# vdBerg93/cl-rrt

Hardware: AMD Instinct MI355X
Metric: nodes expanded/sec (200-obstacle scene) (higher is better)
Workload: dtype f64

## Files before the change

cl-rrt_amd/clrrt/__init__.py:

```python
import ctypes as C
import os

import numpy as np

from . import abi
from .abi import (CLRRT_COLLISION_OBB, CLRRT_COLLISION_STUB, CLRRT_MODE_BATCH,
                  CLRRT_MODE_EXACT, ROLL_NAMES)

PKG_DIR = os.path.dirname(os.path.dirname(os.path.abspath(__file__)))
LIB_PATH = os.environ.get("CLRRT_LIB") or os.path.join(PKG_DIR, "libclrrt.so")
HEADER_PATH = os.path.join(os.path.dirname(PKG_DIR), "include", "clrrt.h")

_lib = None
P = C.POINTER
EXCHANGE_FN = C.CFUNCTYPE(C.c_int32, C.c_void_p, P(abi.ExchangeIO))

_SIGS = {
    "clrrt_abi_version": (C.c_int, []),
    "clrrt_params_default": (C.c_int, [P(abi.Params), C.c_double, P(C.c_double), C.c_double]),
    "clrrt_rng_seed": (None, [P(abi.Rng), C.c_uint32]),
    "clrrt_rng_next": (C.c_int32, [P(abi.Rng)]),
    "clrrt_draw_samples": (C.c_int, [P(abi.Params), P(abi.Rng), C.c_int32, P(abi.Sample)]),
    "clrrt_create": (C.c_int, [P(abi.Params), P(abi.Capacity), C.c_int, P(C.c_void_p)]),
    "clrrt_destroy": (None, [C.c_void_p]),
# ... 486 lines not shown
        self._chk(self.L.clrrt_exact_stats(self.h, out), "exact_stats")
        return dict(zip(("rounds", "resolved", "fixup_rollouts", "conflict_rounds", "end_fixup_succeeded", "end_tie",
                         "end_key_eq_thr", "end_over_slots", "end_pushed_out"), list(out)[:9]))

    def iteration_log(self, on=True):
        self._chk(self.L.clrrt_iteration_log(self.h, 1 if on else 0), "iteration_log")

    def iterations(self):
        n = C.c_int64()
        self._chk(self.L.clrrt_iteration_records(self.h, 0, 0, None, C.byref(n)), "iteration_records")
        arr = (abi.Iteration * max(1, n.value))()
        self._chk(self.L.clrrt_iteration_records(self.h, 0, n.value, arr, C.byref(n)), "iteration_records")
        return {f: np.array([getattr(arr[i], f) for i in range(n.value)], dtype=np.int64)
                for f, _ in abi.Iteration._fields_}

    def round_sizes(self):
        n = C.c_int64()
        self._chk(self.L.clrrt_round_sizes(self.h, None, 0, C.byref(n)), "round_sizes")
        out = np.zeros(max(1, n.value), dtype=np.int64)
        self._chk(self.L.clrrt_round_sizes(self.h, out.ctypes.data_as(P(C.c_int64)), n.value, C.byref(n)), "round_sizes")
        return out[:n.value]

    def walk_audit(self, samples):
        n = len(samples)
        arr = (abi.Sample * n)(*samples)
        out = np.zeros((n, 20), dtype=np.int32)
        self._chk(self.L.clrrt_walk_audit(self.h, arr, n, out.ctypes.data_as(P(C.c_int32))), "walk_audit")
        return out

    def search_work_ex(self):
        out = (C.c_int64 * 8)()
        self._chk(self.L.clrrt_search_work_ex(self.h, out), "search_work_ex")
        return {"bf_keys": out[0], "samples": out[1], "tiles": out[2], "exact_keys": out[3],
                "super_bounds": out[4], "super_visits": out[5], "queued": out[6]}

    def reset_counters(self):
        self._chk(self.L.clrrt_reset_counters(self.h), "reset_counters")

    def enable_timing(self, on=True):
        self._chk(self.L.clrrt_enable_timing(self.h, 1 if on else 0), "enable_timing")

    def set_option(self, key, value):
        self._chk(self.L.clrrt_set_option(self.h, key.encode(), int(value)), f"set_option({key})")

    def nn_stats(self):
        out = (C.c_int64 * 19)()
        self._chk(self.L.clrrt_nn_stats(self.h, out), "nn_stats")
        return {"waves": out[0], "nodes_read": out[1], "rings": out[2], "truncated_waves": out[3],
                "last_fallback_samples": out[4], "tiles_seen": out[5], "tiles_searched": out[6],
                "pairs_queued": out[7], "exact_keys": out[8], "walk_supers": out[10], "walk_tiles": out[11],
                "walk_queued": out[12], "walk_exact": out[13], "walk_clk_bounds": out[14], "walk_clk_super": out[15],
                "walk_clk_visit": out[16], "walk_clk_drain": out[17], "walk_clk_total": out[18]}

    def debug_counters(self):
        out = (C.c_int64 * 64)()
        self._chk(self.L.clrrt_debug_counters(self.h, out), "debug_counters")
        return list(out)

    def kernel_time(self, which):
        ms, n = C.c_double(), C.c_int64()
        self._chk(self.L.clrrt_kernel_time(self.h, which, C.byref(ms), C.byref(n)), "kernel_time")
        return ms.value, n.value
```

cl-rrt_amd/csrc/clrrt_capi.hip:

```cpp
#include <hip/hip_runtime.h>
#include <math.h>

#include <algorithm>
#include <climits>
#include <array>
#include <chrono>
#include <cmath>
#include <cstdio>
#include <cstdlib>
#include <cstring>
#include <deque>
#include <functional>
#include <optional>
#include <string>
#include <vector>

#include "../../include/clrrt.h"
#include "clrrt_dev.hpp"
#include "clrrt_internal.hpp"

static const int kWalkMaxOver = 2048, kWalkMaxChunks = 64;

using namespace clrrt;

// ... 35 lines not shown
  KeyId* sort_scratch = nullptr;
  int64_t sort_cap = 0;
  RollRes* res_spec = nullptr;
  clrrt_node* regnodes = nullptr;
  RollRes* res_gb = nullptr;
  double* slots = nullptr;
  int slot_rows = 0;
  int rows_deferred = 1;
  void* rep_buf = nullptr;
  int rep_n = 0;
  bool eval_deferred = false;
  clrrt_node* gbnodes = nullptr;
  SampleOut* so = nullptr;
  int* first_conflict = nullptr;
  clrrt_node* out_nodes = nullptr;
  Job* jobs = nullptr;
  int64_t* totals = nullptr;
  bool totals_zeroed = false;
  unsigned long long* work_ctr = nullptr;
  float* nn_seed = nullptr;
  double bbox[4] = {HUGE_VAL, HUGE_VAL, -HUGE_VAL, -HUGE_VAL};
  double* d_bbox = nullptr;
  double* h_bbox = nullptr;
  int64_t nnw_min_nodes = 8192;
  bool nnw_stateless = false;
  int nnw_bud_tiles = 3072, nnw_bud_ex = 4096, nnw_chunks = 16, nnw_max_over = 1024;
  bool nnw_max_over_set = false;
  bool nnw_bud_tiles_set = false;
  int nnw_half_max = 4096;
  int nnw_hscale = 50;
  int nnw_lpt = 0;
  int nnw_root_seed = 1;
  int nnw_root_k = 64;
  int nnw_root_scan = 16384;
  int nnw_index = 5;
  int nnw_lds_floor = 0;
  int nnw_waves = -1;
  int nnw_double = 1;
  WalkBufs nnw{};
  WalkBufs nnw_alt{};
  struct { int64_t n = -1; double ox, oy, x0, y0, x1, y1; float delta; } nnw_built;
  CompactBufs cmp{};
  int roll_persistent = 1;
  int nn_debug = 0;
  int roll_blocks = 0;
  int n_cu = 256;
  int* roll_q = nullptr;
  int* roll_best = nullptr;
  int roll_priority = 1;
  int roll_order_verify = 0;
  int roll_coop = 1;
  int roll_spread = 1;
  int roll_lanes = 0;
  int nn_exact_fused = 1;
  int exact_min_width = 8;
  int exact_fixup = 1;
  int exact_fix_cap = 0;
  int* fix_n = nullptr;
  int* fix_ids = nullptr;
  int* fix_adj = nullptr;
  NnRec* fix_xrec = nullptr;
  int* fix_xi = nullptr;
  int* fix_xcand = nullptr;
  float* fix_xkey = nullptr;
  int* fix_xn = nullptr;
  std::vector<int> h_fix_cand;
// ... 1115 lines not shown
  HIPC(c, hipSetDevice(c->device));
  unsigned long long h[4];
  HIPC(c, hipMemcpyAsync(h, c->work_ctr, sizeof(h), hipMemcpyDeviceToHost, c->stream));
  HIPC(c, hipStreamSynchronize(c->stream));
  for (int i = 0; i < 3; i++) out[i] = (int64_t)h[i];
  return CLRRT_OK;
}

int clrrt_search_work(clrrt_ctx* c, int64_t out[4]) {
  if (!c || !out) return CLRRT_EINVAL;
  HIPC(c, hipSetDevice(c->device));
  HIPC(c, hipStreamSynchronize(c->stream));
  if (c->side) HIPC(c, hipStreamSynchronize(c->side));
  unsigned long long h[19];
  HIPC(c, hipMemcpy(h, c->work_ctr + 8, sizeof(h), hipMemcpyDeviceToHost));
  out[0] = c->nn_bf_keys;
  out[1] = c->nn_samples;
  out[2] = (int64_t)h[11];
  out[3] = (int64_t)h[13];
  return CLRRT_OK;
}

int clrrt_search_work_ex(clrrt_ctx* c, int64_t out[8]) {
  if (!c || !out) return CLRRT_EINVAL;
  int64_t w[4];
  const int rc = clrrt_search_work(c, w);
  if (rc != CLRRT_OK) return rc;
  unsigned long long h[19];
  HIPC(c, hipMemcpy(h, c->work_ctr + 8, sizeof(h), hipMemcpyDeviceToHost));
  for (int i = 0; i < 4; i++) out[i] = w[i];
  out[4] = c->nn_super_bounds;
  out[5] = (int64_t)h[10];
  out[6] = (int64_t)h[12];
  out[7] = 0;
  return CLRRT_OK;
}

int clrrt_nn_stats(clrrt_ctx* c, int64_t out[19]) {
  if (!c || !out) return CLRRT_EINVAL;
  HIPC(c, hipSetDevice(c->device));
  HIPC(c, hipStreamSynchronize(c->stream));
  unsigned long long h[19];
  HIPC(c, hipMemcpy(h, c->work_ctr + 8, sizeof(h), hipMemcpyDeviceToHost));
  for (int i = 0; i < 19; i++) out[i] = (int64_t)h[i];
  out[4] &= 0xffffffff;
  return CLRRT_OK;
}

int clrrt_set_option(clrrt_ctx* c, const char* key, int64_t value) {
  if (!c || !key) return CLRRT_EINVAL;
  const std::string k(key);
  if (k == "roll_persistent") c->roll_persistent = value != 0;
  else if (k == "nn_walk_min" && value >= 0) c->nnw_min_nodes = value;
  else if (k == "nn_walk_stateless") c->nnw_stateless = value != 0;
  else if (k == "nn_walk_budget_tiles" && value >= 0 && value < INT_MAX) {
    c->nnw_bud_tiles = (int)value;
    c->nnw_bud_tiles_set = true;
  }
  else if (k == "nn_walk_budget_keys" && value >= 0 && value < INT_MAX) c->nnw_bud_ex = (int)value;
  else if (k == "nn_walk_half_max" && value >= 0 && value < INT_MAX) c->nnw_half_max = (int)value;
  else if (k == "nn_walk_hscale" && value >= 1 && value <= 10000) {
    c->nnw_hscale = (int)value;
    c->nnw_built.n = -1;
    c->nnw.sorted_n = c->nnw_alt.sorted_n = c->nnw3.sorted_n = -1;
  }
  else if (k == "nn_walk_lpt") c->nnw_lpt = value != 0;
  else if (k == "nn_root_seed" || (k == "nn_root_k" && value >= 1 && value <= 64) ||
           (k == "nn_root_scan" && value >= 1 && value <= 32768)) {
    if (k == "nn_root_seed") c->nnw_root_seed = value != 0;
    else if (k == "nn_root_k") c->nnw_root_k = (int)value;
    else c->nnw_root_scan = (int)value;
    c->nnw_built.n = -1;
  }
  else if (k == "nn_walk_index" && value >= 0 && value <= 5) {
    c->nnw_index = (int)value;
    c->nnw_built.n = -1;
    c->nnw.sorted_n = c->nnw_alt.sorted_n = c->nnw3.sorted_n = -1;
  }
  else if (k == "nn_walk_lds_floor" && value >= 0 && value <= 65536) c->nnw_lds_floor = (int)value;
  else if (k == "nn_walk_waves" && value >= -1 && value <= 1 << 20) c->nnw_waves = (int)value;
  else if (k == "nn_walk_chunks" && value >= 1 && value <= kWalkMaxChunks) c->nnw_chunks = (int)value;
  else if (k == "nn_walk_max_over" && value >= 1 && value <= kWalkMaxOver) {
    c->nnw_max_over = (int)value;
    c->nnw_max_over_set = true;
  }
  else if (k == "nn_walk_double") c->nnw_double = value != 0;
  else if (k == "nn_lag" && (value == 0 || value == 1 || value == 2)) c->nn_lag = (int)value;
  else if (k == "nn_delta_walk") c->nn_delta_walk = value != 0 ? 1 : 0;
  else if (k == "nn_delta_verify") c->nn_delta_verify = value != 0 ? 1 : 0;
  else if (k == "nn_delta_early") c->nn_delta_early = value != 0 ? 1 : 0;
  else if (k == "nn_lane_order") c->nn_lane_order = value != 0 ? 1 : 0;
  else if (k == "nn_debug" && value >= 0) c->nn_debug = (int)value;
  else if (k == "fail_at_round" && value >= 0 && value < INT_MAX) c->fail_at_round = (int)value;
  else if (k == "fail_after_exchange" && value >= 0 && value < INT_MAX) c->fail_after_exchange = (int)value;
  else if (k == "shard_hook_world1") c->sh.hook_world1 = value != 0;
  else if (k == "roll_blocks" && value >= 0 && value < (1 << 20)) c->roll_blocks = (int)value;
  else if (k == "nn_pipeline") c->nn_pipeline = value != 0;
  else if (k == "roll_priority") c->roll_priority = value != 0;
  else if (k == "roll_order_verify") c->roll_order_verify = value != 0;
// ... 140 lines not shown
                    : (int)std::max<int64_t>(c->nnw_bud_tiles, c->n_nodes >> 11);
  w.bud_ex = c->nnw_bud_ex > 0 ? (int)std::max<int64_t>(c->nnw_bud_ex, c->n_nodes >> 9) : 0;
  w.max_over = c->nnw_max_over_set || c->n_nodes < (6 << 20) ? c->nnw_max_over : kWalkMaxOver;
  w.nch = c->nnw_chunks;
  w.half_max = c->nnw_half_max;
  w.index_kind = c->nnw_index;
  w.hscale_pct = c->nnw_hscale;
  w.lpt = c->nnw_lpt;
  w.root_seed = c->nnw_root_seed;
  w.root_k = c->nnw_root_k;
  w.root_scan = c->nnw_root_scan;
  w.lds_floor = c->nnw_lds_floor;
  w.waves = c->nnw_waves < 0 ? 9 * c->n_cu : c->nnw_waves;
  w.waves_min_batch = c->nnw_waves < 0 ? 4 * w.waves : 0;
  return alloc_walk(c, w);
}
static int ensure_walk(clrrt_ctx* c) { return ensure_walk_set(c, c->nnw); }

struct NnSetup {
  NnFrame fr;
  double x0, y0, x1, y1;
  bool region_ok;
};
static NnSetup nn_setup(clrrt_ctx* c) {
  NnSetup su;
  double& x0 = su.x0; double& y0 = su.y0; double& x1 = su.x1; double& y1 = su.y1;
  sample_region(c->params, x0, y0, x1, y1);
  if (c->bbox[0] <= c->bbox[2]) {
    x0 = std::min(x0, c->bbox[0] - 1.0); y0 = std::min(y0, c->bbox[1] - 1.0);
    x1 = std::max(x1, c->bbox[2] + 1.0); y1 = std::max(y1, c->bbox[3] + 1.0);
  }
  NnFrame fr;
  fr.debug = c->nn_debug;
  fr.ox = 0.5 * (x0 + x1);
  fr.oy = 0.5 * (y0 + y1);
  {
    const double E = std::max(x1 - x0, y1 - y0) + 1.0;
    const double d = 16.0 * std::ldexp(E, -24) + 1e-5;
    fr.delta = std::isfinite(d) ? (float)d : HUGE_VALF;
  }
  su.fr = fr;
  const double W = x1 - x0, H = y1 - y0;
  su.region_ok = std::isfinite(W * H) && W * H > 0;
  return su;
}

static bool walk_serves(clrrt_ctx* c, const NnSetup& su) {
  return c->n_nodes >= c->nnw_min_nodes && su.region_ok;
}

static void pf_discard(clrrt_ctx* c) {
  if (c->pf_state != 0 && c->side) hipStreamSynchronize(c->side);
  c->pf_state = 0;
  c->pf_next.clear();
}
static void pf_reset(clrrt_ctx* c) {
  pf_discard(c);
  c->nnr_built.n = -1;
  c->nnw_built.n = -1;
  c->nnw.sorted_n = -1;
  c->nnw_alt.sorted_n = -1;
  c->nnw3.sorted_n = -1;
}

static bool walk_built_for(const clrrt_ctx* c, const NnSetup& su) {
  const auto& b = c->nnw_built;
// ... 1937 lines not shown
```

cl-rrt_amd/csrc/clrrt_internal.hpp:

```cpp
#pragma once
#include <hip/hip_runtime.h>
#include <stdint.h>

#include "../../include/clrrt.h"
#include "clrrt_dev.hpp"
#include "clrrt_stdsort.hpp"

namespace clrrt {

#define CLRRT_ROLL_PENDING (-2)

struct RollRes {
  double st[10];
  double costE, costS;
  double bx, by;
  double fx, fy;
  double vback;
  int32_t outcome;
  int32_t nrows;
  int32_t refN;
  int32_t pad;
};

struct WorkCtr {
// ... 76 lines not shown
  void* carry_out;
  int* ncarry_out;
  int carry_cap;
  int jbase, sbase;
  unsigned long long* dbg;
  const clrrt_node* __restrict__ xreg;
  const clrrt_node* __restrict__ xgb;
  int job_stride;
};

struct SelArgs {
  DevParams p;
  const clrrt_node* __restrict__ tree;
  const int* __restrict__ cand;
  const float* __restrict__ ckey;
  const int* __restrict__ ncand;
  const RollRes* __restrict__ res;
  const RollRes* __restrict__ res_gb;
  clrrt_node* regnodes;
  clrrt_node* gbnodes;
  SampleOut* so;
  int B;
  const int* view;
  int nd, sbase;
  int* gv;
  uint8_t* pend;
  int* new_pend;
};

struct NnFrame {
  double ox, oy;
  float delta;
  int debug;
};
struct WalkTile {
  float pcx, pcy, pr;
  float rcx, rcy, rr;
  float thx, thy, thh;
  float apx, apy, aph;
  float cemin;
  float aopt;
  int32_t nonfinite;
  float eroot;
};
static_assert(sizeof(WalkTile) == 64, "WalkTile layout");
struct WalkBufs {
  uint32_t *keys, *keys2;
  int *vals, *vals2;
  int* sorder;
  void* tmp;
  size_t tmp_bytes;
  float4 *P, *Q;
  float* CE;
  int* ID;
  int* HEAD;
  int2* trun;
  WalkTile *tiles, *supers;
  int bud_tiles, bud_ex, max_over, nch;
  int half_max = 4096;
  int lds_floor = 0;
  int waves = 0;
  int waves_min_batch = 0;
  int index_kind = 0;
  int hscale_pct = 100;
  int* wctr = nullptr;
  int* roster = nullptr;
// ... 151 lines not shown
```

cl-rrt_amd/csrc/clrrt_nnwalk.hip:

```cpp
#include <hip/hip_runtime.h>
#include <climits>
#include <hip/hip_fp16.h>
#include <hipcub/hipcub.hpp>
#include <rocprim/device/device_merge.hpp>
#include <algorithm>
#include <stdint.h>

#include "clrrt_dev.hpp"
#include "clrrt_internal.hpp"

namespace clrrt {

#define CAND_K 10
#define NN_K (CAND_K + 1)
#define WALK_TILE 32
#define WALK_SUPER 32
#define WALK_FMT_STATE 0
#define WALK_FMT_HALF 1
#define WALK_FMT_CODED 2
#ifndef WALK_STAGE1_QUEUE
#define WALK_STAGE1_QUEUE 0
#endif
#ifndef WALK_HALF_SUPER
#define WALK_HALF_SUPER 1
#endif
#define WALK_TQ 68
#ifndef WALK_SPLIT_SHARE
#define WALK_SPLIT_SHARE 1
#endif
#ifndef CLRRT_DELTA_ONEPASS
#define CLRRT_DELTA_ONEPASS 1
#endif
#ifndef WALK_APBINS
#define WALK_APBINS 8
#endif
#ifndef WALK_SECTOR_BITS
#define WALK_SECTOR_BITS 3
#endif

#define WALK_ROOT_BIT 0x40000000
#define WALK_ROOT_KMAX 64
#define WALK_ROOT_SMAX 32768

#define LAUNCH_CHECK3()                        \
  do {                                           \
    hipError_t e_ = hipGetLastError();           \
    if (e_ != hipSuccess) return e_;             \
  } while (0)

__device__ __forceinline__ uint32_t w_spread(uint32_t v) {
  v &= 0xffff;
  v = (v | (v << 8)) & 0x00ff00ff;
  v = (v | (v << 4)) & 0x0f0f0f0f;
  v = (v | (v << 2)) & 0x33333333;
  v = (v | (v << 1)) & 0x55555555;
  return v;
}

__device__ __forceinline__ uint64_t w_spread3(uint32_t v) {
  uint64_t x = v & 0xffff;
  x = (x | (x << 16)) & 0x0000ff0000ffull;
  x = (x | (x << 8)) & 0x00f00f00f00full;
  x = (x | (x << 4)) & 0x0c30c30c30c3ull;
  x = (x | (x << 2)) & 0x249249249249ull;
  return x;
}

__global__ void k_walk_keys(const NnRec* __restrict__ nodes, int N, double x0, double y0, double scale,
                            uint64_t* __restrict__ keys, int* __restrict__ vals, int first = 0, int kind = 0,
                            double hrho = 4.77) {
  const int k0 = blockIdx.x * blockDim.x + threadIdx.x;
  if (k0 >= N - first) return;
  const int i = first + k0;
  keys += -first;
  vals += -first;
// ... 338 lines not shown
      const float df2 = tx * tx + (ty + rho) * (ty + rho);
      const float cA = fminf(fmaxf((5.f * rho * rho - df2) * (1.f / (4.f * rho * rho)), -1.f), 1.f);
      const float sA = fsqrt(fmaxf((1.f - cA) * (1.f + cA), 0.f));
      const float u = rho * sA;
      const float w = fsqrt(fmaxf(df2 - u * u, 0.f));
      const float cw = w * frcp(fsqrt(df2));
      if (sA >= 0.05f && cw >= 0.05f) {
        const float alpha = 6.28318531f - atan2_apx(sA, cA);
        const float L = rho * (alpha + atan2_apx(tx, ty + rho) + atan2_apx(u, w));
        const float m = 2e-3f + 1e-4f * L + pos_err * (8.f + 8.f * frcp(sA) + 8.f * frcp(cw));
        lo = fmaxf(L - m, 14.9f);
        hi = L + m;
      }
    }
    return;
  }
  if (!(t2 > -0.01f)) {
    lo = -__builtin_inff();
    hi = __builtin_inff();
    return;
  }
  const float t = fsqrt(fmaxf(t2, 0.f));
  float th = atan2_apx(tx, rho - ty);
  if (th < 0.f) th += 6.28318531f;
  const float L = t + rho * (th - atan2_apx(t, rho));
  const float m = 2.f * pos_err + 2e-4f + 2e-5f * L;
  if (t2 >= 0.01f) {
    lo = L - m;
    hi = L + m;
  } else {
    lo = fminf(L - m - 1e-4f, 14.9f);
    hi = __builtin_inff();
  }
}

__device__ __forceinline__ float walk_lb(const WalkTile& w, float rsx, float rsy, bool ex, float flen,
                                         float dsR = 0.f) {
  if (w.nonfinite) return -__builtin_inff();
  if (w.pr < 0.f) return __builtin_inff();
  const float rho = 4.77f;
  const float ex2 = rsx - w.rcx, ey2 = rsy - w.rcy;
  const float E2 = fsqrt(ex2 * ex2 + ey2 * ey2);
  if (E2 + w.rr < flen) return __builtin_inff();
  if (E2 > w.rr && w.aph < 3.f) {
    const float iE = frcp(E2);
    const float a2 = 1.57079633f - acos_apx(w.rr * iE);
    const float ang2 = acos_apx((ex2 * w.apx + ey2 * w.apy) * iE);
    if (ang2 - a2 - w.aph > 0.78539816f + 5e-3f) return __builtin_inff();
  }
  const float dx = rsx - w.pcx, dy = rsy - w.pcy;
  const float D = fsqrt(dx * dx + dy * dy);
  float lb = D - w.pr;
  if (D > w.pr && w.thh < 3.f) {
    const float iD = frcp(D);
    const float al = 1.57079633f - acos_apx(w.pr * iD);
    const float bmin = acos_apx((dx * w.thx + dy * w.thy) * iD) - al - w.thh - 3e-3f;
    lb = fmaxf(lb, rho * bmin);
  }
  lb = lb - 2e-3f - 1e-5f * fabsf(lb);
  if (!ex) lb = fmaxf(fmaxf(w.aopt + D * (1.f - 1e-5f) - 2e-3f, w.cemin + lb), w.eroot + dsR);
  return lb == lb ? lb : -__builtin_inff();
}

#ifndef WALK_CHEAP_FIRST
#define WALK_CHEAP_FIRST 1
#endif
// ... 145 lines not shown
  float uk = __builtin_inff();
  float kth = __builtin_inff();
  int kth_c = 255;
  float base = 0.f;
  int idk = 0x7fffffff;
  float lim = __builtin_inff();
  float cb0 = -2.f;
  int n2 = 0;
#ifdef CLRRT_WALK_PROFILE
  const bool prof = fr.debug == 2;
#else
  constexpr bool prof = false;
#endif
  uint64_t cyc[4] = {0, 0, 0, 0};
#ifdef CLRRT_WALK_PROFILE
  unsigned long long hist[6] = {0, 0, 0, 0, 0, 0};
#endif
  int hc = -1;
  float kc = 0.f;
  __shared__ int s_root[4];
  int seeded = -1;
  if constexpr (!SPLIT) {
    float kr = -__builtin_inff();
    int rX = -1;
    if (roster && !ex) seeded = walk_root_seed(sx, sy, nodes, roster, p.feas_len, lane, kr, rX, lk, li);
    if (lane == 0) {
      s_root[0] = __float_as_int(kr);
      s_root[1] = rX;
      s_root[2] = seeded;
    }
    __builtin_amdgcn_wave_barrier();
  }
  unsigned long long n_sup = 0, n_tile = 0, n_q = 0, n_ex = 0, n_und = 0, n_sure = 0, n_drop = 0;

  auto refresh = [&]() __attribute__((always_inline)) {
    kth = uni(__shfl(lk, NN_K - 1, 64));
    idk = uni(__shfl(li, NN_K - 1, 64));
    if (SPLIT && w_less(kb, ib, kth, idk)) { kth = kb; idk = ib; }
    const float u10 = uni(__shfl(uk, NN_K - 1, 64));
    if (u10 < kth) { kth = u10; idk = 0x7fffffff; }
#if WALK_SPLIT_SHARE
    if constexpr (SPLIT && SHARE) {
      int* sh = &ovf[o_sp].w;
      if (lane == 0 && kth < __builtin_inff() && !(kth < 0.f)) atomicMin(sh, kth > 0.f ? __float_as_int(kth) : 0);
      const float shv = __int_as_float(uni(__atomic_load_n(sh, __ATOMIC_RELAXED)));
      if (shv < kth) { kth = shv; idk = 0x7fffffff; }
    }
#endif
    if constexpr (CODED) kth_c = uni(lc_le(kth - base));
    if (kth < __builtin_inff()) {
      const float R = (kth + 2e-4f) * (1.0f / 0.9999f);
      lim = uni(R < 0.f ? -1.f : (R + dl) * (R + dl));
      const float b0 = (kth + 0.01f) * (1.f / rho) + 2e-3f;
      cb0 = uni(b0 < 3.1f ? __cosf(b0) - 1e-4f : -2.f);
    }
  };
  auto drain_exact = [&](int room) __attribute__((always_inline)) {
    if (n2 == 0) return;
    {
      const int jj = lane < n2 ? s_q2[lane] : 0;
      const float bb = lane < n2 ? s_b2[lane] : 0.f;
      const bool k2 = lane < n2 && !(bb > kth);
      const uint64_t m2 = __ballot(k2);
      __builtin_amdgcn_wave_barrier();
      if (k2) {
        const int pos = __popcll(m2 & ((1ull << lane) - 1));
        s_q2[pos] = jj;
        s_b2[pos] = bb;
      }
      __builtin_amdgcn_wave_barrier();
      n_drop += n2 - __popcll(m2);
      n2 = __popcll(m2);
      if (n2 == 0 || n2 + room <= 64) return;
    }
    const int nq = n2;
    const uint64_t c0 = prof ? __builtin_amdgcn_s_memtime() : 0;
    n_ex += nq;
    bool c = false;
    float key = 0.f;
    int id = 0, j = 0;
    if (lane < nq) {
      j = s_q2[lane];
      id = ID[j];
      const NnRec& r = nodes[id];
      key = dubins_key(sx, sy, r.x, r.y, r.c, r.s);
      if (!ex) key = r.costE + key;
      if (w_less(key, id, kth, idk)) {
        c = feasible_search(sx, sy, r.bx, r.by, r.ca, r.sa, r.ang_par, p.feas_len);
      }
    }
    {
      const int hd = lane < nq ? HEAD[j] : 0;
      const int depth = lane < nq ? j - (hd & ~WALK_ROOT_BIT) : -1;
      int best = depth;
#pragma unroll
      for (int o = 32; o > 0; o >>= 1) best = max(best, __shfl_xor(best, o, 64));
      best = uni(best);
      if (best > 0) {
        const int l = __ffsll((unsigned long long)__ballot(depth == best)) - 1;
        kc = uni(__shfl(key, l, 64));
        hc = uni(__shfl(hd, l, 64));
      }
    }
#ifdef CLRRT_WALK_PROFILE
    if (prof) {
      const float gap = key - kth;
      const bool v = lane < nq;
      hist[0] += __popcll(__ballot(v && !(gap > 0.f)));
      hist[1] += __popcll(__ballot(v && gap > 0.f && gap <= 1e-3f));
      hist[2] += __popcll(__ballot(v && gap > 1e-3f && gap <= 1e-2f));
      hist[3] += __popcll(__ballot(v && gap > 1e-2f && gap <= 0.1f));
      hist[4] += __popcll(__ballot(v && gap > 0.1f));
      hist[5] += __popcll(__ballot(v && kth == __builtin_inff()));
    }
#endif
    uint64_t m = __ballot(c);
    while (m) {
      const int l = __ffsll((unsigned long long)m) - 1;
      m &= m - 1;
      const float k = __shfl(key, l, 64);
      const int i = __shfl(id, l, 64);
      if (w_less(k, i, kth, idk)) {
        w_insert(lk, li, k, i, lane);
        refresh();
        if constexpr (!SPLIT) {
          if (lane == 0) s_root[2] |= 256;
        }
      }
    }
    n2 = 0;
    if (prof) cyc[3] += __builtin_amdgcn_s_memtime() - c0;
  };
  const float f2_sure = fmaxf((float)(p.feas_len * p.feas_len) * 1.002f + 1e-3f, (1e4f * dl) * (1e4f * dl));
  auto stage1 = [&](bool ok, float4 pp, float4 qq, float ce, float& lbt, float& ubt) __attribute__((always_inline)) {
    lbt = __builtin_inff();
    ubt = __builtin_inff();
    if (!ok) return;
    const float qx = rsx - pp.x, qy = rsy - pp.y;
    const float tx = pp.z * qx - pp.w * qy, ty = fabsf(pp.w * qx + pp.z * qy);
    float lo, hi;
    walk_key_range<BRK>(tx, ty, 4.f * dl + 1e-6f * (fabsf(tx) + ty), lo, hi);
    const float cst = ex ? 0.f : ce;
    const float tlo = cst + lo, thi = cst + hi;
    lbt = tlo - 1e-6f * fabsf(tlo);
    const float vx = rsx - qq.x, vy = rsy - qq.y;
    const float dot = vx * qq.z + vy * qq.w, vv = vx * vx + vy * vy;
    const bool sure = dot > 0.f && dot * dot >= 0.502f * vv && vv >= f2_sure;
    ubt = sure ? thi + 1e-6f * fabsf(thi) : __builtin_inff();
  };
  auto ub_insert = [&](float ubt) __attribute__((always_inline)) {
    uint64_t mu = __ballot(ubt < kth);
    if (!mu) return false;
    while (mu) {
      const int l = __ffsll((unsigned long long)mu) - 1;
      mu &= mu - 1;
      const float v = __shfl(ubt, l, 64);
      const float u10 = uni(__shfl(uk, NN_K - 1, 64));
      if (v < u10) {
        const int pos = __popcll(__ballot(uk <= v && lane < NN_K));
        const float up = __shfl_up(uk, 1, 64);
        if (lane < NN_K) {
          if (lane == pos) uk = v;
          else if (lane > pos) uk = up;
        }
      }
    }
    return true;
  };
  auto enqueue = [&](bool ok, float lbt, int j) __attribute__((always_inline)) {
    const bool keep = ok && !(lbt > kth);
    const uint64_t m = __ballot(keep);
    const int cnt = __popcll(m);
    if (cnt == 0) return;
    if (n2 + cnt > 64) drain_exact(cnt);
    __builtin_amdgcn_wave_barrier();
    if (keep) {
      const int pos = n2 + __popcll(m & ((1ull << lane) - 1));
      s_q2[pos] = j;
      s_b2[pos] = lbt;
    }
    n2 += cnt;
    __builtin_amdgcn_wave_barrier();
  };
  auto drain = [&]() __attribute__((always_inline)) { drain_exact(64); };
  auto prefilter = [&](int id, int hd, float4 pp, float4 qq, float ce) __attribute__((always_inline)) -> bool {
    if (hd == hc && !w_less(kc, id, kth, idk)) return false;
    if constexpr (!SPLIT) {
      if (hd & WALK_ROOT_BIT) {
        if (id <= s_root[1] || !w_less(__int_as_float(s_root[0]), id, kth, idk)) return false;
      }
    }
    const float qx = rsx - pp.x, qy = rsy - pp.y;
    const float d2 = qx * qx + qy * qy;
    float l2 = lim;
    if (!ex) {
      const float R = (kth - ce + 2e-4f) * (1.0f / 0.9999f);
      l2 = R < 0.f ? -1.f : (R + dl) * (R + dl);
    }
    if (!(id >= 0 && ((d2 <= l2) || (l2 != l2)))) return false;
    const float vx = rsx - qq.x, vy = rsy - qq.y;
    const float dot = vx * qq.z + vy * qq.w, vv = vx * vx + vy * vy;
    const bool ang_bad = (vv < fl2) || (dot < -1e-3f) || (dot * dot < c45 * c45 * vv && dot >= 0.f);
    const float tx = pp.z * qx - pp.w * qy, ty = fabsf(pp.w * qx + pp.z * qy);
    const bool deep = tx * tx + (ty - rho) * (ty - rho) <= rin2;
    const bool in_bad = deep && !(ex ? (14.9f <= kth) : (ce + 14.9f <= kth));
    bool turn_bad = false;
    if (ex) {
      if (cb0 > -1.5f) {
        const float qn = fsqrt(d2);
        turn_bad = tx + 4.f * dl + 1e-6f * qn < cb0 * qn;
      }
    } else if (kth < __builtin_inff()) {
      const float b0 = (kth - ce + 0.01f) * (1.f / rho) + 2e-3f;
      if (b0 < 3.1f) {
        const float cb = __cosf(b0) - 1e-4f;
        const float qn = fsqrt(d2);
        turn_bad = tx + 4.f * dl + 1e-6f * qn < cb * qn;
      }
    }
    return !ang_bad && !in_bad && !turn_bad;
  };
#if WALK_STAGE1_QUEUE
  int n1 = 0;
  auto push1 = [&](bool ok, int j) __attribute__((always_inline)) {
    const uint64_t m = __ballot(ok);
    if (ok) s_q1[n1 + __popcll(m & ((1ull << lane) - 1))] = j;
    n1 += __popcll(m);
    __builtin_amdgcn_wave_barrier();
  };
  auto run_stage1 = [&](int cnt) __attribute__((always_inline)) {
    const int b0 = n1 - cnt;
    const bool v = lane < cnt;
    const int j = v ? s_q1[b0 + lane] : -1;
    __builtin_amdgcn_wave_barrier();
    n1 = b0;
    float4 pp = make_float4(0.f, 0.f, 1.f, 0.f), qq = pp;
    float ce = 0.f;
    if (v) { pp = P[j]; qq = Q[j]; ce = CE[j]; }
    float lt, ut;
    stage1(v, pp, qq, ce, lt, ut);
    n_und += __popcll(__ballot(lt == -__builtin_inff()));
    n_sure += __popcll(__ballot(ut < __builtin_inff()));
    if (ub_insert(ut)) refresh();
    enqueue(v, lt, j);
  };
#endif
  auto visit4 = [&](int t0, int t1, int t2, int t3) __attribute__((always_inline)) {
    const uint64_t c0 = prof ? __builtin_amdgcn_s_memtime() : 0;
    n_tile += (t0 >= 0) + (t1 >= 0) + (t2 >= 0) + (t3 >= 0);
    const int ta = lane < 32 ? t0 : t1, tb = lane < 32 ? t2 : t3;
    const int ja = ta >= 0 ? ta * WALK_TILE + (lane & 31) : -1;
    const int jb = tb >= 0 ? tb * WALK_TILE + (lane & 31) : -1;
    int ida = -1, idb = -1, ha = -2, hb = -2;
    float4 pa = make_float4(0.f, 0.f, 1.f, 0.f), qa = pa, pb = pa, qb = pa;
    float ca = 0.f, cb = 0.f;
    if (ja >= 0) { ida = ID[ja]; ha = HEAD[ja]; pa = P[ja]; qa = Q[ja]; ca = CE[ja]; }
    if (jb >= 0) { idb = ID[jb]; hb = HEAD[jb]; pb = P[jb]; qb = Q[jb]; cb = CE[jb]; }
    const bool oka = prefilter(ida, ha, pa, qa, ca);
    const bool okb = prefilter(idb, hb, pb, qb, cb);
    n_q += __popcll(__ballot(oka)) + __popcll(__ballot(okb));
#if WALK_STAGE1_QUEUE
    push1(oka, ja);
    push1(okb, jb);
    while (n1 >= 64) run_stage1(64);
#else
    float la, ua, lb, ub;
    stage1(oka, pa, qa, ca, la, ua);
    stage1(okb, pb, qb, cb, lb, ub);
    n_und += __popcll(__ballot(la == -__builtin_inff())) + __popcll(__ballot(lb == -__builtin_inff()));
    n_sure += __popcll(__ballot(ua < __builtin_inff())) + __popcll(__ballot(ub < __builtin_inff()));
    const bool ia = ub_insert(ua);
    const bool ib2 = ub_insert(ub);
    if (ia || ib2) refresh();
    enqueue(oka, la, ja);
    enqueue(okb, lb, jb);
#endif
    if (prof) cyc[2] += __builtin_amdgcn_s_memtime() - c0;
  };
  auto hmin = [&](float v) -> float {
#pragma unroll
    for (int o = 16; o > 0; o >>= 1) v = fminf(v, __shfl_xor(v, o, 64));
    return v;
  };
  auto run_out = [&](int tl) -> bool {
    const int2 tr = trun[tl];
    if constexpr (!SPLIT) {
      if (tr.x >= 0 && (tr.x & WALK_ROOT_BIT) && !w_less(__int_as_float(s_root[0]), tr.y, kth, idk)) return true;
    }
    return tr.x >= 0 && tr.x == hc && !w_less(kc, tr.y, kth, idk);
  };
  int qn = 0;
  auto next_q = [&]() __attribute__((always_inline)) -> int {
    while (qn > 0) {
      qn--;
      const int t = uni(s_tq[qn]);
      if (!(uni(s_tb[qn]) > kth)) return t;
    }
    return -1;
  };
  auto visit_queue = [&]() __attribute__((always_inline)) {
    const int t0 = next_q();
    const int t1 = next_q();
    const int t2 = next_q();
    const int t3 = next_q();
    if (t0 >= 0) visit4(t0, t1, t2, t3);
    __builtin_amdgcn_wave_barrier();
  };
  auto flush_queue = [&]() __attribute__((always_inline)) {
// ... 55 lines not shown
      if (st >= 0 && tl < ntiles) lb = fmaxf(walk_lb(tiles[tl], rsx, rsy, ex, flen_t, dsR), slb);
#endif
      if (st >= 0 && tl < ntiles && run_out(tl)) lb = __builtin_inff();
      const bool take = st >= 0 && (first || lb > Tp) && lb <= T && !(lb > kth);
      tm = __ballot(take);
      const float rest = hmin(st >= 0 && lb > T ? lb : __builtin_inff());
      if ((lane & 31) == 0 && st >= 0) {
        if constexpr (CODED) s_lb[lo] = (uint8_t)lc_enc(rest - base);
        else s_lbh[lo] = __float2half_rd(rest);
      }
    }
    const bool tk = (tm >> lane) & 1ull;
    if (tk) {
      const int pos = qn + __popcll(tm & ((1ull << lane) - 1));
      s_tq[pos] = st * WALK_SUPER + (lane & 31);
      s_tb[pos] = lb;
    }
    qn += __popcll(tm);
    __builtin_amdgcn_wave_barrier();
    while (qn >= 4) visit_queue();
    if (prof) cyc[1] += __builtin_amdgcn_s_memtime() - c0;
  };

  const uint64_t ct0 = prof ? __builtin_amdgcn_s_memtime() : 0;
  auto flush_stats = [&]() {
    if (stats && lane == 0) {
      atomicAdd(&stats[0], n_sup);
      atomicAdd(&stats[1], n_tile);
      atomicAdd(&stats[2], n_q);
      atomicAdd(&stats[3], n_ex);
      atomicAdd(&stats[10], n_und);
      atomicAdd(&stats[11], n_sure);
      atomicAdd(&stats[12], n_drop);
      if (prof) {
        atomicAdd(&stats[4], (unsigned long long)cyc[0]);
        atomicAdd(&stats[5], (unsigned long long)cyc[1]);
        atomicAdd(&stats[6], (unsigned long long)cyc[2]);
        atomicAdd(&stats[7], (unsigned long long)cyc[3]);
        atomicAdd(&stats[8], (unsigned long long)(__builtin_amdgcn_s_memtime() - ct0));
#ifdef CLRRT_WALK_PROFILE
        atomicAdd(&stats[13], hist[0]);
        for (int q = 1; q < 6; q++) atomicAdd(&stats[14 + q], hist[q]);
#endif
      }
    }
  };
  if (SPLIT) refresh();
  if constexpr (!SPLIT) {
    if (seeded >= 0) refresh();
  }
  float mlb = __builtin_inff();
  for (int t0 = 0; t0 < nloc; t0 += 64) {
    const int t = t0 + lane;
    if (t < nloc) {
      const float lb = walk_lb(sup[gst(t)], rsx, rsy, ex, flen_t, dsR);
      if constexpr (STATE) {
        s_lbf[t] = lb;
        s_vis[t] = 0u;
      } else if constexpr (!CODED) {
        s_lbh[t] = __float2half_rd(lb);
        if constexpr (WALK_HALF_SUPER) s_sh[t] = s_lbh[t];
      }
      mlb = fminf(mlb, lb);
    }
  }
  mlb = wmin(mlb);
  base = mlb > 0.f && mlb < __builtin_inff() ? mlb : 0.f;
  if constexpr (CODED) {
    for (int t0 = 0; t0 < nloc; t0 += 64) {
      const int t = t0 + lane;
      if (t < nloc) s_lb[t] = (uint8_t)lc_enc(walk_lb(sup[gst(t)], rsx, rsy, ex, flen_t, dsR) - base);
    }
  }
  __builtin_amdgcn_wave_barrier();
  if (prof) cyc[0] += __builtin_amdgcn_s_memtime() - ct0;
// ... 4 lines not shown
#define WALK_GROW 2.f
#endif
  float T = base + WALK_T0, Tp = -__builtin_inff();
#if CLRRT_DELTA_ONEPASS
  if constexpr (SPLIT && !SHARE) {
    if (kb < __builtin_inff()) T = __builtin_inff();
  }
#endif
  bool budget = !SPLIT && (bud_tiles > 0 || bud_ex > 0);
  for (int pass = 0;; pass++) {
    const float lim_t = fminf(T, kth);
    const int lim_c = CODED ? uni(lc_le(lim_t - base)) : 0;
    for (int t0 = 0; t0 < nloc; t0 += 64) {
      const int t = t0 + lane;
      bool want;
      if constexpr (CODED) {
        const int c = t < nloc ? s_lb[t] : 255;
        want = c != 255 && c <= lim_c;
      } else {
        const float lb = t < nloc ? (STATE ? s_lbf[t] : __half2float(s_lbh[t])) : __builtin_inff();
        want = lb < __builtin_inff() && lb <= lim_t;
      }
      uint64_t m = __ballot(want);
      while (m) {
        int sa = -1, sb = -1;
        while (m && sb < 0) {
          const int st = t0 + __ffsll((unsigned long long)m) - 1;
          m &= m - 1;
          if (CODED ? (int)s_lb[st] > kth_c : (STATE ? s_lbf[st] : __half2float(s_lbh[st])) > kth) continue;
          if (sa < 0) sa = st; else sb = st;
        }
        if (sa >= 0) visit_supers(sa, sb, Tp, T, pass == 0);
        if (budget && ((bud_tiles > 0 && n_tile > (unsigned long long)bud_tiles) ||
                       (bud_ex > 0 && n_ex > (unsigned long long)bud_ex))) {
          int slot = 0;
          if (lane == 0) slot = atomicAdd(ovf_n, 1);
          slot = uni(__shfl(slot, 0, 64));
          if (slot < max_over) {
            if (lane == 0)
              ovf[slot] = make_int4(s, __float_as_int(kth), idk == 0x7fffffff ? idk : idk + 1,
                                    kth > 0.f ? __float_as_int(kth) : kth == 0.f ? 0 : 0x7f800000);
            if (stats && lane == 0) atomicAdd(&stats[14], 1ull);
            flush_stats();
            return;
          }
          budget = false;
        }
      }
    }
    flush_queue();
    drain();
    if (T == __builtin_inff() || kth <= T) break;
    Tp = T;
    T = base + (T - base) * WALK_GROW;
    if (T > 1e7f) T = __builtin_inff();
  }
  if constexpr (SPLIT) {
    const int o = o_sp;
    if (lane < NN_K) {
      pk[((size_t)o * nch + ch) * NN_K + lane] = lk;
      pi[((size_t)o * nch + ch) * NN_K + lane] = li;
    }
  } else {
    walk_emit(lk, li, lane, s, p.sort_limit, cand, ckey, ncand, ctie);
    if (stats && lane == 0) {
      const int seed_st = s_root[2];
      if (seed_st > 0 && seed_st < 256) atomicAdd(&stats[9], 1ull);
// ... 628 lines not shown
```

Measured before the change: 1.477 million.

## Tighten drain-time bounds for query-inside-turning-circle candidates before exact Dubins keys

Stage 1 now marks queued candidates whose query point lies inside the node's turning circle, where the bracket lower bound is loose. At drain time those flagged candidates get a tighter inside-case lower bound, and any that exceed the current kth are dropped before the costly exact Dubins key evaluation. Dropped candidates can still seed the run-out memo, and they count toward the exact-key budget. This adds extra per-drain ballots and loads, and it is on by default through a new option.

```diff
diff --git a/cl-rrt_amd/clrrt/__init__.py b/cl-rrt_amd/clrrt/__init__.py
--- a/cl-rrt_amd/clrrt/__init__.py
+++ b/cl-rrt_amd/clrrt/__init__.py
@@ -542,7 +542,7 @@
         out = (C.c_int64 * 8)()
         self._chk(self.L.clrrt_search_work_ex(self.h, out), "search_work_ex")
         return {"bf_keys": out[0], "samples": out[1], "tiles": out[2], "exact_keys": out[3],
-                "super_bounds": out[4], "super_visits": out[5], "queued": out[6]}
+                "super_bounds": out[4], "super_visits": out[5], "queued": out[6], "bracket_drops": out[7]}
 
     def reset_counters(self):
         self._chk(self.L.clrrt_reset_counters(self.h), "reset_counters")
diff --git a/cl-rrt_amd/csrc/clrrt_capi.hip b/cl-rrt_amd/csrc/clrrt_capi.hip
--- a/cl-rrt_amd/csrc/clrrt_capi.hip
+++ b/cl-rrt_amd/csrc/clrrt_capi.hip
@@ -91,6 +91,7 @@
   int nnw_lpt = 0;
   int nnw_root_seed = 1;
   int nnw_root_k = 64;
+  int nnw_drain_brk = 1;
   int nnw_root_scan = 16384;
   int nnw_index = 5;
   int nnw_lds_floor = 0;
@@ -1272,7 +1273,9 @@
   out[4] = c->nn_super_bounds;
   out[5] = (int64_t)h[10];
   out[6] = (int64_t)h[12];
-  out[7] = 0;
+  unsigned long long brk = 0;
+  HIPC(c, hipMemcpy(&brk, c->work_ctr + 49, sizeof(brk), hipMemcpyDeviceToHost));
+  out[7] = (int64_t)brk;
   return CLRRT_OK;
 }
 
@@ -1305,6 +1308,7 @@
     c->nnw.sorted_n = c->nnw_alt.sorted_n = c->nnw3.sorted_n = -1;
   }
   else if (k == "nn_walk_lpt") c->nnw_lpt = value != 0;
+  else if (k == "nn_drain_bracket") c->nnw_drain_brk = value != 0;
   else if (k == "nn_root_seed" || (k == "nn_root_k" && value >= 1 && value <= 64) ||
            (k == "nn_root_scan" && value >= 1 && value <= 32768)) {
     if (k == "nn_root_seed") c->nnw_root_seed = value != 0;
@@ -1511,6 +1515,7 @@
   }
   NnFrame fr;
   fr.debug = c->nn_debug;
+  fr.drain_brk = c->nnw_drain_brk;
   fr.ox = 0.5 * (x0 + x1);
   fr.oy = 0.5 * (y0 + y1);
   {
diff --git a/cl-rrt_amd/csrc/clrrt_internal.hpp b/cl-rrt_amd/csrc/clrrt_internal.hpp
--- a/cl-rrt_amd/csrc/clrrt_internal.hpp
+++ b/cl-rrt_amd/csrc/clrrt_internal.hpp
@@ -132,6 +132,7 @@
   double ox, oy;
   float delta;
   int debug;
+  int drain_brk = 1;
 };
 struct WalkTile {
   float pcx, pcy, pr;
diff --git a/cl-rrt_amd/csrc/clrrt_nnwalk.hip b/cl-rrt_amd/csrc/clrrt_nnwalk.hip
--- a/cl-rrt_amd/csrc/clrrt_nnwalk.hip
+++ b/cl-rrt_amd/csrc/clrrt_nnwalk.hip
@@ -41,6 +41,10 @@
 #define WALK_ROOT_BIT 0x40000000
 #define WALK_ROOT_KMAX 64
 #define WALK_ROOT_SMAX 32768
+#define WALK_Q2_INSIDE 0x40000000
+#ifndef WALK_DROP_MEMO
+#define WALK_DROP_MEMO 1
+#endif
 
 #define LAUNCH_CHECK3()                        \
   do {                                           \
@@ -445,6 +449,12 @@
     lo = fminf(L - m - 1e-4f, 14.9f);
     hi = __builtin_inff();
   }
+}
+
+__device__ __forceinline__ float walk_inside_lo(float tx, float ty, float pos_err) {
+  float lo, hi;
+  walk_key_range<true>(tx, ty, pos_err, lo, hi);
+  return lo;
 }
 
 __device__ __forceinline__ float walk_lb(const WalkTile& w, float rsx, float rsy, bool ex, float flen,
@@ -656,6 +666,7 @@
     __builtin_amdgcn_wave_barrier();
   }
   unsigned long long n_sup = 0, n_tile = 0, n_q = 0, n_ex = 0, n_und = 0, n_sure = 0, n_drop = 0;
+  unsigned int n_brk = 0;
 
   auto refresh = [&]() __attribute__((always_inline)) {
     kth = uni(__shfl(lk, NN_K - 1, 64));
@@ -697,6 +708,54 @@
       n2 = __popcll(m2);
       if (n2 == 0 || n2 + room <= 64) return;
     }
+    int mdep = 0;
+    if constexpr (!BRK) {
+      const int jq = lane < n2 ? s_q2[lane] : 0;
+      const bool fl = (jq & WALK_Q2_INSIDE) != 0;
+      if (__ballot(fl)) {
+        const uint64_t c0 = prof ? __builtin_amdgcn_s_memtime() : 0;
+        const int j = jq & ~WALK_Q2_INSIDE;
+        float bb = lane < n2 ? s_b2[lane] : 0.f;
+        if (fl) {
+          const float4 pp = P[j];
+          const float cst = ex ? 0.f : CE[j];
+          const float qx = rsx - pp.x, qy = rsy - pp.y;
+          const float tx = pp.z * qx - pp.w * qy, ty = fabsf(pp.w * qx + pp.z * qy);
+          const float tlo = cst + walk_inside_lo(tx, ty, 4.f * dl + 1e-6f * (fabsf(tx) + ty));
+          bb = tlo - 1e-6f * fabsf(tlo);
+        }
+        const bool k3 = lane < n2 && !(bb > kth);
+        const uint64_t m3 = __ballot(k3);
+#if WALK_DROP_MEMO
+        {
+          const bool dr = fl && !k3;
+          const int hd = dr ? HEAD[j] : 0;
+          const int depth = dr ? j - (hd & ~WALK_ROOT_BIT) : -1;
+          int best = depth;
+#pragma unroll
+          for (int o = 32; o > 0; o >>= 1) best = max(best, __shfl_xor(best, o, 64));
+          best = uni(best);
+          if (best > 0) {
+            const int l = __ffsll((unsigned long long)__ballot(depth == best)) - 1;
+            kc = uni(__shfl(bb, l, 64));
+            hc = uni(__shfl(hd, l, 64));
+            mdep = best;
+          }
+        }
+#endif
+        __builtin_amdgcn_wave_barrier();
+        if (k3) {
+          const int pos = __popcll(m3 & ((1ull << lane) - 1));
+          s_q2[pos] = j;
+          s_b2[pos] = bb;
+        }
+        __builtin_amdgcn_wave_barrier();
+        n_brk += n2 - __popcll(m3);
+        n2 = __popcll(m3);
+        if (prof) cyc[3] += __builtin_amdgcn_s_memtime() - c0;
+        if (n2 == 0 || n2 + room <= 64) return;
+      }
+    }
     const int nq = n2;
     const uint64_t c0 = prof ? __builtin_amdgcn_s_memtime() : 0;
     n_ex += nq;
@@ -704,7 +763,7 @@
     float key = 0.f;
     int id = 0, j = 0;
     if (lane < nq) {
-      j = s_q2[lane];
+      j = s_q2[lane] & ~WALK_Q2_INSIDE;
       id = ID[j];
       const NnRec& r = nodes[id];
       key = dubins_key(sx, sy, r.x, r.y, r.c, r.s);
@@ -720,7 +779,7 @@
 #pragma unroll
       for (int o = 32; o > 0; o >>= 1) best = max(best, __shfl_xor(best, o, 64));
       best = uni(best);
-      if (best > 0) {
+      if (best > 0 && best >= mdep) {
         const int l = __ffsll((unsigned long long)__ballot(depth == best)) - 1;
         kc = uni(__shfl(key, l, 64));
         hc = uni(__shfl(hd, l, 64));
@@ -756,14 +815,18 @@
     if (prof) cyc[3] += __builtin_amdgcn_s_memtime() - c0;
   };
   const float f2_sure = fmaxf((float)(p.feas_len * p.feas_len) * 1.002f + 1e-3f, (1e4f * dl) * (1e4f * dl));
-  auto stage1 = [&](bool ok, float4 pp, float4 qq, float ce, float& lbt, float& ubt) __attribute__((always_inline)) {
+  auto stage1 = [&](bool ok, float4 pp, float4 qq, float ce, float& lbt, float& ubt, bool& ins) __attribute__((always_inline)) {
     lbt = __builtin_inff();
     ubt = __builtin_inff();
+    ins = false;
     if (!ok) return;
     const float qx = rsx - pp.x, qy = rsy - pp.y;
     const float tx = pp.z * qx - pp.w * qy, ty = fabsf(pp.w * qx + pp.z * qy);
     float lo, hi;
     walk_key_range<BRK>(tx, ty, 4.f * dl + 1e-6f * (fabsf(tx) + ty), lo, hi);
+    if constexpr (!BRK) {
+      ins = fr.drain_brk && tx * tx + ty * (ty - 2.f * rho) <= -0.01f;
+    }
     const float cst = ex ? 0.f : ce;
     const float tlo = cst + lo, thi = cst + hi;
     lbt = tlo - 1e-6f * fabsf(tlo);
@@ -791,7 +854,7 @@
     }
     return true;
   };
-  auto enqueue = [&](bool ok, float lbt, int j) __attribute__((always_inline)) {
+  auto enqueue = [&](bool ok, float lbt, int j, bool ins) __attribute__((always_inline)) {
     const bool keep = ok && !(lbt > kth);
     const uint64_t m = __ballot(keep);
     const int cnt = __popcll(m);
@@ -800,7 +863,7 @@
     __builtin_amdgcn_wave_barrier();
     if (keep) {
       const int pos = n2 + __popcll(m & ((1ull << lane) - 1));
-      s_q2[pos] = j;
+      s_q2[pos] = ins ? j | WALK_Q2_INSIDE : j;
       s_b2[pos] = lbt;
     }
     n2 += cnt;
@@ -862,11 +925,12 @@
     float ce = 0.f;
     if (v) { pp = P[j]; qq = Q[j]; ce = CE[j]; }
     float lt, ut;
-    stage1(v, pp, qq, ce, lt, ut);
+    bool in1;
+    stage1(v, pp, qq, ce, lt, ut, in1);
     n_und += __popcll(__ballot(lt == -__builtin_inff()));
     n_sure += __popcll(__ballot(ut < __builtin_inff()));
     if (ub_insert(ut)) refresh();
-    enqueue(v, lt, j);
+    enqueue(v, lt, j, in1);
   };
 #endif
   auto visit4 = [&](int t0, int t1, int t2, int t3) __attribute__((always_inline)) {
@@ -889,15 +953,16 @@
     while (n1 >= 64) run_stage1(64);
 #else
     float la, ua, lb, ub;
-    stage1(oka, pa, qa, ca, la, ua);
-    stage1(okb, pb, qb, cb, lb, ub);
+    bool ina, inb;
+    stage1(oka, pa, qa, ca, la, ua, ina);
+    stage1(okb, pb, qb, cb, lb, ub, inb);
     n_und += __popcll(__ballot(la == -__builtin_inff())) + __popcll(__ballot(lb == -__builtin_inff()));
     n_sure += __popcll(__ballot(ua < __builtin_inff())) + __popcll(__ballot(ub < __builtin_inff()));
     const bool ia = ub_insert(ua);
     const bool ib2 = ub_insert(ub);
     if (ia || ib2) refresh();
-    enqueue(oka, la, ja);
-    enqueue(okb, lb, jb);
+    enqueue(oka, la, ja, ina);
+    enqueue(okb, lb, jb, inb);
 #endif
     if (prof) cyc[2] += __builtin_amdgcn_s_memtime() - c0;
   };
@@ -1019,6 +1084,7 @@
       atomicAdd(&stats[10], n_und);
       atomicAdd(&stats[11], n_sure);
       atomicAdd(&stats[12], n_drop);
+      if (n_brk) atomicAdd(&stats[SPLIT && !SHARE ? 9 : 31], (unsigned long long)n_brk);
       if (prof) {
         atomicAdd(&stats[4], (unsigned long long)cyc[0]);
         atomicAdd(&stats[5], (unsigned long long)cyc[1]);
@@ -1028,6 +1094,12 @@
 #ifdef CLRRT_WALK_PROFILE
         atomicAdd(&stats[13], hist[0]);
         for (int q = 1; q < 6; q++) atomicAdd(&stats[14 + q], hist[q]);
+        if constexpr (SPLIT && SHARE) {
+          for (int q = 0; q < 4; q++) atomicAdd(&stats[22 + q], (unsigned long long)cyc[q]);
+          atomicAdd(&stats[26], (unsigned long long)(__builtin_amdgcn_s_memtime() - ct0));
+          atomicAdd(&stats[27], n_ex);
+          for (int q = 0; q < 6; q++) atomicAdd(&stats[32 + q], hist[q]);
+        }
 #endif
       }
     }
@@ -1098,7 +1170,7 @@
         }
         if (sa >= 0) visit_supers(sa, sb, Tp, T, pass == 0);
         if (budget && ((bud_tiles > 0 && n_tile > (unsigned long long)bud_tiles) ||
-                       (bud_ex > 0 && n_ex > (unsigned long long)bud_ex))) {
+                       (bud_ex > 0 && n_ex + n_brk > (unsigned long long)bud_ex))) {
           int slot = 0;
           if (lane == 0) slot = atomicAdd(ovf_n, 1);
           slot = uni(__shfl(slot, 0, 64));
```

After: 1.501 million, median of 4. 1.02x the previous value.
